# aliabdelkader/FusionTransformer

Measured on AMD Instinct MI355X. Metric: frames/sec fwd+bwd (SemanticKITTI synth), whole job, higher is better.
Workload: dtype f32

## Files before the change

fusiontransformer_amd/csrc/ftx_bn.hip:

```cpp
#include <cstdlib>
#include <map>
#include <mutex>
#include <utility>
#include "ftx_common.h"
#include "ftx_bn_eval_op.h"
#include "ftx_lastblock.h"

using namespace ftx;

namespace ftx {
namespace {
struct ScratchEntry {
  StreamScratch sc;
  void *owned;
};
std::mutex g_scratch_mu;
std::map<std::pair<int, hipStream_t>, ScratchEntry> g_scratch;

constexpr size_t scratch_counter_bytes() { return 512 * ((sizeof(uint32_t) * (1 + LB_MAX_GROUPS) + 511) / 512); }
constexpr size_t scratch_group_bytes() { return sizeof(double) * (size_t)LB_MAX_GROUPS * 2 * LB_MAX_COLS; }

int current_device() {
  int dev = 0;
  if (hipGetDevice(&dev) != hipSuccess) (void)hipGetLastError();
  return dev;
}
}

StreamScratch stream_scratch(hipStream_t st) {
  std::lock_guard<std::mutex> lock(g_scratch_mu);
  const auto key = std::make_pair(current_device(), st);
  auto it = g_scratch.find(key);
  if (it != g_scratch.end()) return it->second.sc;
  StreamScratch sc{nullptr, nullptr};
  hipStreamCaptureStatus cap = hipStreamCaptureStatusNone;
  if (hipStreamIsCapturing(st, &cap) == hipSuccess && cap != hipStreamCaptureStatusNone) {
    set_error("stream_scratch: first use of a stream inside a capture (attach a buffer, or run the op once on that stream, before capturing)");
    return sc;
  }
  (void)hipGetLastError();
  char *base = nullptr;
  if (hipMalloc((void **)&base, scratch_counter_bytes() + scratch_group_bytes()) != hipSuccess ||
      hipMemsetAsync(base, 0, scratch_counter_bytes(), st) != hipSuccess) {
    set_error("stream_scratch: cannot allocate the per-stream ticket buffer (%s)", hipGetErrorString(hipGetLastError()));
    if (base) (void)hipFree(base);
    return sc;
  }
  sc.counters = (uint32_t *)base;
  sc.gpart = (double *)(base + scratch_counter_bytes());
  g_scratch[key] = ScratchEntry{sc, base};
  return sc;
}
}

extern "C" size_t ftx_stream_scratch_bytes(void) { return scratch_counter_bytes() + scratch_group_bytes(); }

extern "C" int ftx_stream_scratch_attach(void *stream, void *buffer, size_t bytes) {
  FTX_REQUIRE(buffer && ((uintptr_t)buffer & 255) == 0, "ftx_stream_scratch_attach: the buffer must be non-null and 256-byte aligned");
  FTX_REQUIRE(bytes >= ftx_stream_scratch_bytes(), "ftx_stream_scratch_attach: %zu bytes < ftx_stream_scratch_bytes() = %zu", bytes, ftx_stream_scratch_bytes());
  hipStream_t st = (hipStream_t)stream;
  std::lock_guard<std::mutex> lock(g_scratch_mu);
  const auto key = std::make_pair(current_device(), st);
  if (hipMemsetAsync(buffer, 0, scratch_counter_bytes(), st) != hipSuccess) return check_launch("ftx_stream_scratch_attach memset");
  auto it = g_scratch.find(key);
  if (it != g_scratch.end() && it->second.owned) {
    if (hipStreamSynchronize(st) != hipSuccess) (void)hipGetLastError();
    (void)hipFree(it->second.owned);
  }
  StreamScratch sc{(uint32_t *)buffer, (double *)((char *)buffer + scratch_counter_bytes())};
  g_scratch[key] = ScratchEntry{sc, nullptr};
  return FTX_OK;
}

extern "C" int ftx_stream_scratch_reset(void *stream) {
  hipStream_t st = (hipStream_t)stream;
  std::lock_guard<std::mutex> lock(g_scratch_mu);
  auto it = g_scratch.find(std::make_pair(current_device(), st));
  if (it == g_scratch.end()) return FTX_OK;
  if (hipMemsetAsync(it->second.sc.counters, 0, scratch_counter_bytes(), st) != hipSuccess) return check_launch("ftx_stream_scratch_reset");
  return FTX_OK;
}

extern "C" int ftx_stream_scratch_release(void *stream) {
  hipStream_t st = (hipStream_t)stream;
  std::lock_guard<std::mutex> lock(g_scratch_mu);
  auto it = g_scratch.find(std::make_pair(current_device(), st));
  if (it == g_scratch.end()) return FTX_OK;
  if (hipStreamSynchronize(st) != hipSuccess) (void)hipGetLastError();
  if (it->second.owned) (void)hipFree(it->second.owned);
  g_scratch.erase(it);
  return FTX_OK;
}

static int bn_blocks(int64_t n) {
  constexpr int rows = 48, maxb = 2048;
  int64_t b = ceil_div(n, rows);
  if (b > maxb) b = maxb;
  if (b > LB_GROUP * LB_MAX_GROUPS) b = LB_GROUP * LB_MAX_GROUPS;
  if (b < 1) b = 1;
  return (int)b;
}

extern "C" size_t ftx_bn_workspace_bytes(int64_t n, int32_t c) {
  if (c <= 0) return 256;
  return sizeof(double) * (size_t)bn_blocks(n) * 2 * c + sizeof(double) * 2 * c;
}

__device__ inline float bn_affine(float x, float mean, float invstd, float gamma, float beta) {
  return __fmaf_rn(__fmul_rn(__fsub_rn(x, mean), invstd), gamma, beta);
}

struct FwdOp {
  __device__ static void eval(float x, float, float, float, float, float, float, int, double &q0, double &q1) {
    q0 = (double)x;
    q1 = (double)x * (double)x;
  }
};
struct BwdOp {
  __device__ static void eval(float x, float gy, float y, float mean, float invstd, float gamma, float beta, int relu, double &q0, double &q1) {
    if (relu == 2) y = bn_affine(x, mean, invstd, gamma, beta);
    float dy = (relu && !(y > 0.f)) ? 0.f : gy;
    q0 = (double)dy;
    q1 = (double)dy * (double)((x - mean) * invstd);
  }
};

template <class Op>
__global__ __launch_bounds__(256) void bn_partial_kernel(const float *__restrict__ x, const float *__restrict__ gy,
                                                         const float *__restrict__ y, const float *__restrict__ mean,
                                                         const float *__restrict__ invstd, const float *__restrict__ gamma,
                                                         const float *__restrict__ beta, int relu, int64_t n, int c,
                                                         double *part, StreamScratch sc) {
  extern __shared__ double sh[];
  const int c4 = c >> 2;
  const int RL = 256 / c4 > 0 ? 256 / c4 : 1;
  const int tid = threadIdx.x;
  const int cg = tid % c4, rl = tid / c4;
  const int64_t rows_per_block = ceil_div(n, (int64_t)gridDim.x);
  const int64_t r0 = (int64_t)blockIdx.x * rows_per_block;
  const int64_t r1 = (r0 + rows_per_block < n) ? r0 + rows_per_block : n;
  double s0[4] = {0, 0, 0, 0}, s1[4] = {0, 0, 0, 0};
  if (rl < RL) {
    float4 mu = make_float4(0, 0, 0, 0), is = mu, gm = mu, bt = mu;
    if (mean) {
      mu = *(const float4 *)&mean[cg * 4];
      is = *(const float4 *)&invstd[cg * 4];
    }
    if (relu == 2) {
      gm = *(const float4 *)&gamma[cg * 4];
      bt = *(const float4 *)&beta[cg * 4];
    }
    auto accumulate = [&](const float4 &xv, const float4 &gv, const float4 &yv) {
      double a, b;
      Op::eval(xv.x, gv.x, yv.x, mu.x, is.x, gm.x, bt.x, relu, a, b); s0[0] += a; s1[0] += b;
      Op::eval(xv.y, gv.y, yv.y, mu.y, is.y, gm.y, bt.y, relu, a, b); s0[1] += a; s1[1] += b;
      Op::eval(xv.z, gv.z, yv.z, mu.z, is.z, gm.z, bt.z, relu, a, b); s0[2] += a; s1[2] += b;
      Op::eval(xv.w, gv.w, yv.w, mu.w, is.w, gm.w, bt.w, relu, a, b); s0[3] += a; s1[3] += b;
    };
    const float4 zero4 = make_float4(0, 0, 0, 0);
    int64_t r = r0 + rl;
    for (; r + RL < r1; r += 2 * RL) {
      const int64_t o0 = r * c + cg * 4, o1 = (r + RL) * c + cg * 4;
      const float4 xa = *(const float4 *)&x[o0], xb = *(const float4 *)&x[o1];
      const float4 ga = gy ? *(const float4 *)&gy[o0] : zero4, gb = gy ? *(const float4 *)&gy[o1] : zero4;
      const float4 ya = y ? *(const float4 *)&y[o0] : zero4, yb = y ? *(const float4 *)&y[o1] : zero4;
      accumulate(xa, ga, ya);
      accumulate(xb, gb, yb);
    }
    for (; r < r1; r += RL) {
      const int64_t o0 = r * c + cg * 4;
      accumulate(*(const float4 *)&x[o0], gy ? *(const float4 *)&gy[o0] : zero4, y ? *(const float4 *)&y[o0] : zero4);
    }
#pragma unroll
    for (int v = 0; v < 4; ++v) {
      sh[(0 * RL + rl) * c + cg * 4 + v] = s0[v];
      sh[(1 * RL + rl) * c + cg * 4 + v] = s1[v];
    }
  }
  __syncthreads();
  for (int j = tid; j < 2 * c; j += 256) {
    int which = j / c, col = j - which * c;
    double s = 0;
    for (int q = 0; q < RL; ++q) s += sh[(which * RL + q) * c + col];
    lb_store(&part[((int64_t)blockIdx.x * 2 + which) * c + col], s);
  }
  __syncthreads();
  last_block_totals(part, (int)gridDim.x, c, sc, sh, StoreTotals{part + (int64_t)gridDim.x * 2 * c, c});
}

__device__ inline void bn_column_stats(double s, double ss, int64_t n, float eps, float &mean, float &invstd, double &var_out) {
  const double m = s / (double)n;
  double var = ss / (double)n - m * m;
  if (var < 0) var = 0;
  mean = (float)m;
  invstd = (float)(1.0 / sqrt(var + (double)eps));
  var_out = var;
}

__global__ __launch_bounds__(256) void bn_apply_fwd_kernel(const float *__restrict__ x, const float *__restrict__ res, const float *__restrict__ gamma,
                                                           const float *__restrict__ beta, const double *__restrict__ totals, float eps,
                                                           float momentum, float *__restrict__ running_mean, float *__restrict__ running_var,
                                                           float *__restrict__ save_mean, float *__restrict__ save_invstd, int64_t n, int c,
                                                           int relu, float *__restrict__ y) {
  const int c4 = c >> 2;
  const int RL = 256 / c4 > 0 ? 256 / c4 : 1;
  const int cg = threadIdx.x % c4, rl = threadIdx.x / c4;
  if (rl >= RL) return;
  const int col = cg * 4;
  float mu_[4], is_[4];
#pragma unroll
  for (int v = 0; v < 4; ++v) {
    double var;
    bn_column_stats(totals[col + v], totals[c + col + v], n, eps, mu_[v], is_[v], var);
    if (blockIdx.x == 0 && rl == 0) {
      save_mean[col + v] = mu_[v];
      save_invstd[col + v] = is_[v];
      if (running_mean) running_mean[col + v] = (1.f - momentum) * running_mean[col + v] + momentum * mu_[v];
      if (running_var) {
        const double unbiased = n > 1 ? var * (double)n / (double)(n - 1) : var;
        running_var[col + v] = (1.f - momentum) * running_var[col + v] + momentum * (float)unbiased;
      }
    }
  }
  const float4 mu = make_float4(mu_[0], mu_[1], mu_[2], mu_[3]), is = make_float4(is_[0], is_[1], is_[2], is_[3]);
  const float4 g = *(const float4 *)&gamma[col], b = *(const float4 *)&beta[col];
  auto one = [&](int64_t r) {
    const int64_t o = r * c + col;
    const float4 xv = *(const float4 *)&x[o];
    float4 ov;
    ov.x = bn_affine(xv.x, mu.x, is.x, g.x, b.x);
    ov.y = bn_affine(xv.y, mu.y, is.y, g.y, b.y);
    ov.z = bn_affine(xv.z, mu.z, is.z, g.z, b.z);
    ov.w = bn_affine(xv.w, mu.w, is.w, g.w, b.w);
    if (res) {
      const float4 rv = *(const float4 *)&res[o];
      ov.x += rv.x; ov.y += rv.y; ov.z += rv.z; ov.w += rv.w;
    }
    if (relu) {
      ov.x = ov.x > 0.f ? ov.x : 0.f; ov.y = ov.y > 0.f ? ov.y : 0.f;
      ov.z = ov.z > 0.f ? ov.z : 0.f; ov.w = ov.w > 0.f ? ov.w : 0.f;
    }
    *(float4 *)&y[o] = ov;
  };
  const int64_t stride = (int64_t)gridDim.x * RL;
  int64_t r = (int64_t)blockIdx.x * RL + rl;
  for (; r + stride < n; r += 2 * stride) {
    one(r);
    one(r + stride);
  }
  if (r < n) one(r);
}

static unsigned bn_apply_grid(int64_t n, int c) {
  const int c4 = c / 4;
  const int rl = 256 / c4 > 0 ? 256 / c4 : 1;
  int64_t g = ceil_div(n, 2 * (int64_t)rl);
  if (g > 4096) g = 4096;
  return (unsigned)(g < 1 ? 1 : g);
}

static int bn_check(const char *who, int64_t n, int c) {
  FTX_REQUIRE(n >= 0, "%s: n < 0", who);
  FTX_REQUIRE(c >= 4 && c % 4 == 0 && c <= 1024, "%s: c must be a multiple of 4 in [4,1024] (got %d)", who, c);
  return FTX_OK;
}

static size_t bn_partial_lds(int c) {
  int c4 = c / 4;
  int RL = 256 / c4 > 0 ? 256 / c4 : 1;
  return sizeof(double) * 2 * RL * c;
}

extern "C" int ftx_bn_train_fwd(const float *x, const float *residual, const float *gamma, const float *beta, float *running_mean,
                                float *running_var, float momentum, float eps, int64_t n, int32_t c, int32_t relu, float *y,
                                float *save_mean, float *save_invstd, void *workspace, size_t workspace_bytes, void *stream) {
  int rc = bn_check("ftx_bn_train_fwd", n, c);
  if (rc != FTX_OK) return rc;
  FTX_REQUIRE(n >= 1, "ftx_bn_train_fwd: needs at least one row");
  FTX_REQUIRE(x && gamma && beta && y && save_mean && save_invstd && workspace, "ftx_bn_train_fwd: null pointer");
  FTX_REQUIRE(c <= 512, "ftx_bn_train_fwd: c > 512 unsupported");
  if (workspace_bytes < ftx_bn_workspace_bytes(n, c)) {
    set_error("ftx_bn_train_fwd: workspace %zu < required %zu", workspace_bytes, ftx_bn_workspace_bytes(n, c));
    return FTX_EWORKSPACE;
  }
  hipStream_t st = (hipStream_t)stream;
  const StreamScratch sc = stream_scratch(st);
  if (!sc.counters) return FTX_ELAUNCH;
  const int nb = bn_blocks(n);
  double *part = (double *)workspace;
  bn_partial_kernel<FwdOp><<<nb, 256, bn_partial_lds(c), st>>>(x, nullptr, nullptr, nullptr, nullptr, nullptr, nullptr, 0, n, c, part, sc);
  bn_apply_fwd_kernel<<<bn_apply_grid(n, c), 256, 0, st>>>(x, residual, gamma, beta, part + (size_t)nb * 2 * c, eps, momentum, running_mean,
                                                           running_var, save_mean, save_invstd, n, c, relu, y);
  return check_launch("ftx_bn_train_fwd");
}

extern "C" int ftx_bn_train_fwd_totals(const float *x, const float *residual, const float *gamma, const float *beta, float *running_mean,
                                       float *running_var, float momentum, float eps, int64_t n, int32_t c, int32_t relu, float *y,
                                       float *save_mean, float *save_invstd, const double *totals, void *stream) {
  int rc = bn_check("ftx_bn_train_fwd_totals", n, c);
  if (rc != FTX_OK) return rc;
  FTX_REQUIRE(n >= 1, "ftx_bn_train_fwd_totals: needs at least one row");
  FTX_REQUIRE(x && gamma && beta && y && save_mean && save_invstd && totals, "ftx_bn_train_fwd_totals: null pointer");
  bn_apply_fwd_kernel<<<bn_apply_grid(n, c), 256, 0, (hipStream_t)stream>>>(x, residual, gamma, beta, totals, eps, momentum, running_mean,
                                                                            running_var, save_mean, save_invstd, n, c, relu, y);
  return check_launch("ftx_bn_train_fwd_totals");
}

__global__ void bn_apply_eval_kernel(const float *__restrict__ x, const float *__restrict__ res, const float *__restrict__ gamma,
                                     const float *__restrict__ beta, const float *__restrict__ rm, const float *__restrict__ rv, float eps,
                                     int64_t n, int c, int relu, float *__restrict__ y) {
  const int c4 = c >> 2;
  const int64_t total = n * c4;
  for (int64_t e = blockIdx.x * (int64_t)blockDim.x + threadIdx.x; e < total; e += (int64_t)gridDim.x * blockDim.x) {
    int col = (int)(e % c4) * 4;
    float4 xv = *(const float4 *)&x[e * 4];
    float o[4] = {xv.x, xv.y, xv.z, xv.w};
    float rr[4] = {0, 0, 0, 0};
    if (res) {
      float4 t = *(const float4 *)&res[e * 4];
      rr[0] = t.x; rr[1] = t.y; rr[2] = t.z; rr[3] = t.w;
    }
#pragma unroll
    for (int v = 0; v < 4; ++v) o[v] = bn_eval_elem(o[v], rm[col + v], rv[col + v], eps, gamma[col + v], beta[col + v], rr[v], relu);
    *(float4 *)&y[e * 4] = make_float4(o[0], o[1], o[2], o[3]);
  }
}

extern "C" int ftx_bn_eval_fwd(const float *x, const float *residual, const float *gamma, const float *beta, const float *running_mean,
                               const float *running_var, float eps, int64_t n, int32_t c, int32_t relu, float *y, void *stream) {
  int rc = bn_check("ftx_bn_eval_fwd", n, c);
  if (rc != FTX_OK) return rc;
  if (n == 0) return FTX_OK;
  FTX_REQUIRE(x && gamma && beta && running_mean && running_var && y, "ftx_bn_eval_fwd: null pointer");
  bn_apply_eval_kernel<<<grid_for(n * (c / 4), 256), 256, 0, (hipStream_t)stream>>>(x, residual, gamma, beta, running_mean, running_var, eps,
                                                                                     n, c, relu, y);
  return check_launch("ftx_bn_eval_fwd");
}

__global__ __launch_bounds__(256) void bn_apply_bwd_kernel(const float *__restrict__ gy, const float *__restrict__ x, const float *__restrict__ y,
                                                           const float *__restrict__ gamma, const float *__restrict__ beta,
                                                           const float *__restrict__ mean,
                                                           const float *__restrict__ invstd, const double *__restrict__ sums, int64_t n, int c,
                                                           int relu, float *__restrict__ gx, float *__restrict__ gres,
                                                           float *__restrict__ grad_gamma, float *__restrict__ grad_beta) {
  const int c4 = c >> 2;
  const int RL = 256 / c4 > 0 ? 256 / c4 : 1;
  const int cg = threadIdx.x % c4, rl = threadIdx.x / c4;
  if (rl >= RL) return;
  const int col = cg * 4;
  const float inv_n = 1.f / (float)n;
  float mu[4], is[4], gm[4], bt[4], sdy[4], sdyx[4];
#pragma unroll
  for (int v = 0; v < 4; ++v) {
    mu[v] = mean[col + v];
    is[v] = invstd[col + v];
    gm[v] = gamma[col + v];
    bt[v] = relu == 2 ? beta[col + v] : 0.f;
    sdy[v] = (float)sums[col + v] * inv_n;
    sdyx[v] = (float)sums[c + col + v] * inv_n;
    if (blockIdx.x == 0 && rl == 0) {
      if (grad_beta) grad_beta[col + v] = (float)sums[col + v];
      if (grad_gamma) grad_gamma[col + v] = (float)sums[c + col + v];
    }
  }
  auto one = [&](int64_t r) {
    const int64_t o = r * c + col;
    const float4 g4 = *(const float4 *)&gy[o];
    const float4 x4 = *(const float4 *)&x[o];
    float dy[4] = {g4.x, g4.y, g4.z, g4.w};
    const float xv[4] = {x4.x, x4.y, x4.z, x4.w};
    if (relu == 2) {
#pragma unroll
      for (int v = 0; v < 4; ++v)
        if (!(bn_affine(xv[v], mu[v], is[v], gm[v], bt[v]) > 0.f)) dy[v] = 0.f;
    } else if (relu) {
      const float4 y4 = *(const float4 *)&y[o];
      const float yv[4] = {y4.x, y4.y, y4.z, y4.w};
#pragma unroll
      for (int v = 0; v < 4; ++v)
        if (!(yv[v] > 0.f)) dy[v] = 0.f;
    }
    float ov[4];
#pragma unroll
    for (int v = 0; v < 4; ++v) {
      const float xhat = (xv[v] - mu[v]) * is[v];
      ov[v] = gm[v] * is[v] * (dy[v] - sdy[v] - xhat * sdyx[v]);
    }
    *(float4 *)&gx[o] = make_float4(ov[0], ov[1], ov[2], ov[3]);
    if (gres) *(float4 *)&gres[o] = make_float4(dy[0], dy[1], dy[2], dy[3]);
  };
  const int64_t stride = (int64_t)gridDim.x * RL;
  int64_t r = (int64_t)blockIdx.x * RL + rl;
  for (; r + stride < n; r += 2 * stride) {
    one(r);
    one(r + stride);
  }
  if (r < n) one(r);
}

extern "C" int ftx_bn_train_bwd(const float *grad_y, const float *x, const float *y, const float *gamma, const float *beta, const float *save_mean,
                                const float *save_invstd, int64_t n, int32_t c, int32_t relu, float *grad_x, float *grad_residual,
                                float *grad_gamma, float *grad_beta, void *workspace, size_t workspace_bytes, void *stream) {
  int rc = bn_check("ftx_bn_train_bwd", n, c);
  if (rc != FTX_OK) return rc;
  FTX_REQUIRE(n >= 1, "ftx_bn_train_bwd: needs at least one row");
  FTX_REQUIRE(grad_y && x && gamma && save_mean && save_invstd && grad_x && workspace, "ftx_bn_train_bwd: null pointer");
  const bool remask = relu && beta != nullptr && grad_residual == nullptr;
  FTX_REQUIRE(!relu || remask || y, "ftx_bn_train_bwd: relu needs the forward output y (or beta, when no residual went into it)");
  const int rmode = !relu ? 0 : (remask ? 2 : 1);
  FTX_REQUIRE(c <= 512, "ftx_bn_train_bwd: c > 512 unsupported");
  if (workspace_bytes < ftx_bn_workspace_bytes(n, c)) {
    set_error("ftx_bn_train_bwd: workspace %zu < required %zu", workspace_bytes, ftx_bn_workspace_bytes(n, c));
    return FTX_EWORKSPACE;
  }
  hipStream_t st = (hipStream_t)stream;
  const StreamScratch sc = stream_scratch(st);
  if (!sc.counters) return FTX_ELAUNCH;
  const int nb = bn_blocks(n);
  double *part = (double *)workspace;
  double *sums = part + (size_t)nb * 2 * c;
  bn_partial_kernel<BwdOp><<<nb, 256, bn_partial_lds(c), st>>>(x, grad_y, rmode == 1 ? y : nullptr, save_mean, save_invstd, gamma, beta, rmode, n, c, part, sc);
  bn_apply_bwd_kernel<<<bn_apply_grid(n, c), 256, 0, st>>>(grad_y, x, y, gamma, beta, save_mean, save_invstd, sums, n, c, rmode, grad_x, grad_residual,
                                                           grad_gamma, grad_beta);
  return check_launch("ftx_bn_train_bwd");
}

struct ColsumGeom {
  int c4w, rl, slab, chunks;
};
static ColsumGeom colsum_geom(int64_t rows, int cols) {
  ColsumGeom g;
  const int c4 = (cols + 3) / 4;
  g.c4w = c4 < 64 ? c4 : 64;
  g.rl = 256 / g.c4w;
  g.slab = g.c4w * 4;
  int64_t ch = ceil_div(rows, (int64_t)g.rl * 8);
  if (ch > 256) ch = 256;
  g.chunks = (int)(ch < 1 ? 1 : ch);
  return g;
}
extern "C" size_t ftx_colsum_workspace_bytes(int64_t rows, int32_t cols) {
  if (rows <= 0 || cols <= 0) return 256;
  return sizeof(double) * (size_t)colsum_geom(rows, cols).chunks * (size_t)cols + 256;
}

__global__ __launch_bounds__(256) void colsum_partial_kernel(const float *__restrict__ x, int64_t rows, int cols, int c4w, int RL,
                                                             double *__restrict__ part) {
  __shared__ double sh[1024];
  const int slab = c4w * 4;
  const int cq = threadIdx.x % c4w, rl = threadIdx.x / c4w;
  const int col = blockIdx.x * slab + cq * 4;
  const int64_t per = ceil_div(rows, (int64_t)gridDim.y);
  const int64_t r0 = (int64_t)blockIdx.y * per, r1 = r0 + per < rows ? r0 + per : rows;
  if (rl < RL) {
    double s[4] = {0, 0, 0, 0};
    if (col < cols) {
      int64_t r = r0 + rl;
      for (; r + RL < r1; r += 2 * RL) {
        const float4 a = *(const float4 *)&x[r * cols + col], b = *(const float4 *)&x[(r + RL) * cols + col];
        s[0] += (double)a.x; s[1] += (double)a.y; s[2] += (double)a.z; s[3] += (double)a.w;
        s[0] += (double)b.x; s[1] += (double)b.y; s[2] += (double)b.z; s[3] += (double)b.w;
      }
      for (; r < r1; r += RL) {
        const float4 a = *(const float4 *)&x[r * cols + col];
        s[0] += (double)a.x; s[1] += (double)a.y; s[2] += (double)a.z; s[3] += (double)a.w;
      }
    }
#pragma unroll
    for (int v = 0; v < 4; ++v) sh[rl * slab + cq * 4 + v] = s[v];
  }
  __syncthreads();
  for (int j = threadIdx.x; j < slab; j += 256) {
    const int c = blockIdx.x * slab + j;
    if (c < cols) {
      double t = 0;
      for (int q = 0; q < RL; ++q) t += sh[q * slab + j];
      part[(int64_t)blockIdx.y * cols + c] = t;
    }
  }
}
// ... 36 lines not shown
```

fusiontransformer_amd/csrc/ftx_lastblock.h:

```cpp
#pragma once
#include <assert.h>
#include "ftx_common.h"

#if defined(__HIP_DEVICE_COMPILE__) && !defined(__gfx950__) && !defined(__gfx942__) && !defined(__gfx90a__)
#error "ftx_lastblock.h relies on gfx9 (CDNA) memory-instruction semantics: sc1 write-through stores and vmcnt-counted store acknowledgements"
#endif

namespace ftx {

constexpr int LB_GROUP = 32;
constexpr int LB_MAX_GROUPS = 128;
constexpr int LB_MAX_COLS = 512;

struct StreamScratch {
  uint32_t *counters;
  double *gpart;
};
StreamScratch stream_scratch(hipStream_t st);

__device__ inline void lb_store(double *p, double v) { __hip_atomic_store(p, v, __ATOMIC_RELAXED, __HIP_MEMORY_SCOPE_AGENT); }
__device__ inline double lb_load(const double *p) { return __hip_atomic_load(p, __ATOMIC_RELAXED, __HIP_MEMORY_SCOPE_AGENT); }
__device__ inline uint32_t lb_ticket(uint32_t *p) { return __hip_atomic_fetch_add(p, 1u, __ATOMIC_RELAXED, __HIP_MEMORY_SCOPE_AGENT); }
__device__ inline void lb_stores_done() {
  asm volatile("s_waitcnt vmcnt(0)" ::: "memory");
  __syncthreads();
}

__device__ inline void lb_column_sums(const double *src, int nrows, int c2, double *slices, double *tot) {
  const int tid = threadIdx.x;
  auto strided_sum = [&](int j, int first, int step) {
    double s = 0;
    for (int base = first; base < nrows; base += 8 * step) {
      double v[8];
#pragma unroll
      for (int u = 0; u < 8; ++u) {
        const int r = base + u * step;
        v[u] = lb_load(&src[(int64_t)(r < nrows ? r : first) * c2 + j]);
        if (r >= nrows) v[u] = 0.0;
      }
#pragma unroll
      for (int u = 0; u < 8; ++u) s += v[u];
    }
    return s;
  };
  if (c2 <= 128) {
    const int R = 256 / c2, j = tid % c2, r = tid / c2;
    if (r < R) slices[r * c2 + j] = strided_sum(j, r, R);
    __syncthreads();
    if (tid < c2) {
      double t = 0;
      for (int q = 0; q < R; ++q) t += slices[q * c2 + tid];
      tot[tid] = t;
    }
  } else {
    for (int j = tid; j < c2; j += 256) tot[j] = strided_sum(j, 0, 1);
  }
  __syncthreads();
}

template <class Fin>
__device__ inline void last_block_totals(const double *part, int nb, int c, StreamScratch sc, double *lds, Fin fin) {
  __shared__ int s_last;
  const int tid = threadIdx.x, c2 = 2 * c;
  const int group = blockIdx.x / LB_GROUP, ngroups = (nb + LB_GROUP - 1) / LB_GROUP;
  const int g0 = group * LB_GROUP;
  const int gsize = nb - g0 < LB_GROUP ? nb - g0 : LB_GROUP;
  double *slices = lds, *tot = lds + 256;
  lb_stores_done();
  if (tid == 0) {
    const uint32_t ticket = lb_ticket(&sc.counters[1 + group]);
    assert(ticket < (uint32_t)gsize && "ftx: dirty BatchNorm ticket (a kernel died on this stream? call ftx_stream_scratch_reset)");
    s_last = ticket == (uint32_t)gsize - 1u;
  }
  __syncthreads();
  if (!s_last) return;
  lb_column_sums(part + (int64_t)g0 * c2, gsize, c2, slices, tot);
  for (int j = tid; j < c2; j += 256) lb_store(&sc.gpart[(int64_t)group * c2 + j], tot[j]);
  lb_stores_done();
  if (tid == 0) {
    __hip_atomic_store(&sc.counters[1 + group], 0u, __ATOMIC_RELAXED, __HIP_MEMORY_SCOPE_AGENT);
    const uint32_t ticket = lb_ticket(&sc.counters[0]);
    assert(ticket < (uint32_t)ngroups && "ftx: dirty BatchNorm group ticket (call ftx_stream_scratch_reset)");
    s_last = ticket == (uint32_t)ngroups - 1u;
  }
  __syncthreads();
  if (!s_last) return;
  if (tid == 0) __hip_atomic_store(&sc.counters[0], 0u, __ATOMIC_RELAXED, __HIP_MEMORY_SCOPE_AGENT);
  lb_column_sums(sc.gpart, ngroups, c2, slices, tot);
  for (int col = tid; col < c; col += 256) fin(col, tot[col], tot[c + col]);
}

struct StoreTotals {
  double *totals;
  int c;
  __device__ void operator()(int col, double s, double ss) const {
    totals[col] = s;
    totals[c + col] = ss;
  }
};

}
```

fusiontransformer_amd/csrc/ftx_spconv.hip:

```cpp
#include <cstring>
#include <cstdlib>
#include "ftx_common.h"
#include "ftx_bn_eval_op.h"
#include "ftx_mfma.h"
#include <rocprim/device/device_scan.hpp>
#include <rocprim/iterator/transform_iterator.hpp>

using namespace ftx;

struct IsValid {
  __host__ __device__ int32_t operator()(int32_t v) const { return v >= 0 ? 1 : 0; }
};

extern "C" size_t ftx_kernel_map_count_workspace_bytes(int64_t n_out, int32_t k) {
  if (n_out <= 0 || k <= 0) return 256;
  size_t bytes = 0;
  const int32_t *in = nullptr;
  int32_t *out = nullptr;
  auto it = rocprim::make_transform_iterator(in, IsValid());
  if (rocprim::exclusive_scan(nullptr, bytes, it, out, 0, (size_t)(n_out * k), rocprim::plus<int32_t>()) != hipSuccess) return 0;
  return bytes + 256;
}

__global__ void koff_kernel(const int32_t *__restrict__ nbr, const int32_t *__restrict__ scan, int64_t n_out, int k, int32_t *__restrict__ koff) {
// ... 442 lines not shown
  if (kvol == 27)
    spconv_reduce_bn_eval_kernel<27><<<(unsigned)g, 256, 0, st>>>(tmp, pos, n, co, residual, gamma, beta, running_mean, running_var, eps, relu, out);
  else
    spconv_reduce_bn_eval_kernel<8><<<(unsigned)g, 256, 0, st>>>(tmp, pos, n, co, residual, gamma, beta, running_mean, running_var, eps, relu, out);
  return check_launch("ftx_spconv_reduce_bn_eval");
}

template <int KVOL>
__global__ __launch_bounds__(256) void spconv_reduce_stats_kernel(const float *__restrict__ tmp, const int32_t *__restrict__ pos, int64_t n, int co,
                                                                  int kvol, float *__restrict__ out, double *part, StreamScratch sc) {
  extern __shared__ double sh[];
  const int cv = co >> 2;
  const int RL = 256 / cv;
  const int tid = threadIdx.x;
  const int cg = tid % cv, rl = tid / cv;
  const int64_t rows_per_block = ceil_div(n, (int64_t)gridDim.x);
  const int64_t r0 = (int64_t)blockIdx.x * rows_per_block;
  const int64_t r1 = (r0 + rows_per_block < n) ? r0 + rows_per_block : n;
  double s0[4] = {0, 0, 0, 0}, s1[4] = {0, 0, 0, 0};
  if (rl < RL) {
    const int j = cg * 4;
    for (int64_t r = r0 + rl; r < r1; r += RL) {
      float4 acc = make_float4(0.f, 0.f, 0.f, 0.f);
      if (KVOL > 0) {
        int32_t p[KVOL > 0 ? KVOL : 1];
#pragma unroll
        for (int k = 0; k < KVOL; ++k) p[k] = pos[(int64_t)k * n + r];
#pragma unroll
        for (int k = 0; k < KVOL; ++k) {
          if (p[k] >= 0) {
            float4 v = *(const float4 *)&tmp[(int64_t)p[k] * co + j];
            acc.x += v.x; acc.y += v.y; acc.z += v.z; acc.w += v.w;
          }
        }
      } else {
        for (int k = 0; k < kvol; ++k) {
          int32_t q = pos[(int64_t)k * n + r];
          if (q >= 0) {
            float4 v = *(const float4 *)&tmp[(int64_t)q * co + j];
            acc.x += v.x; acc.y += v.y; acc.z += v.z; acc.w += v.w;
          }
        }
      }
      *(float4 *)&out[r * co + j] = acc;
      s0[0] += (double)acc.x; s1[0] += (double)acc.x * (double)acc.x;
      s0[1] += (double)acc.y; s1[1] += (double)acc.y * (double)acc.y;
      s0[2] += (double)acc.z; s1[2] += (double)acc.z * (double)acc.z;
      s0[3] += (double)acc.w; s1[3] += (double)acc.w * (double)acc.w;
    }
#pragma unroll
    for (int v = 0; v < 4; ++v) {
      sh[(0 * RL + rl) * co + j + v] = s0[v];
      sh[(1 * RL + rl) * co + j + v] = s1[v];
    }
  }
  __syncthreads();
  for (int e = tid; e < 2 * co; e += 256) {
    int which = e / co, col = e - which * co;
    double s = 0;
    for (int q = 0; q < RL; ++q) s += sh[(which * RL + q) * co + col];
    lb_store(&part[((int64_t)blockIdx.x * 2 + which) * co + col], s);
  }
  __syncthreads();
  last_block_totals(part, (int)gridDim.x, co, sc, sh, StoreTotals{part + (int64_t)gridDim.x * 2 * co, co});
}

extern "C" int32_t ftx_spconv_reduce_stats_blocks(int64_t n, int32_t co) {
  if (n <= 0 || co < 4) return 1;
  const int rl = 256 / (co / 4) > 0 ? 256 / (co / 4) : 1;
  int64_t b = ceil_div(n, 2 * rl);
  if (b > 2048) b = 2048;
  return (int32_t)(b < 1 ? 1 : b);
}

extern "C" int ftx_spconv_reduce_stats(const float *tmp, const int32_t *pos, int64_t n, int32_t co, int32_t kvol, float *out, double *part,
                                       int32_t nb, void *stream) {
  FTX_REQUIRE(n >= 1 && kvol >= 1 && co >= 4 && co % 4 == 0 && co <= 512, "ftx_spconv_reduce_stats: bad size (co must be a multiple of 4 in [4, 512])");
  FTX_REQUIRE(pos && out && part, "ftx_spconv_reduce_stats: null pointer");
  FTX_REQUIRE(nb == ftx_spconv_reduce_stats_blocks(n, co), "ftx_spconv_reduce_stats: nb must come from ftx_spconv_reduce_stats_blocks");
  hipStream_t st = (hipStream_t)stream;
  const StreamScratch sc = stream_scratch(st);
  if (!sc.counters) return FTX_ELAUNCH;
  const int rl = 256 / (co / 4);
  const size_t lds = sizeof(double) * 2 * rl * co;
  if (kvol == 27)
    spconv_reduce_stats_kernel<27><<<nb, 256, lds, st>>>(tmp, pos, n, co, kvol, out, part, sc);
  else if (kvol == 8)
    spconv_reduce_stats_kernel<8><<<nb, 256, lds, st>>>(tmp, pos, n, co, kvol, out, part, sc);
  else
    spconv_reduce_stats_kernel<0><<<nb, 256, lds, st>>>(tmp, pos, n, co, kvol, out, part, sc);
  return check_launch("ftx_spconv_reduce_stats");
}

constexpr int WG_BR = 32;
constexpr int WG_ROUND = 1024;

template <int N> struct FragLoad;
template <> struct FragLoad<1> { static __device__ __forceinline__ void ld(const float *p, float (&f)[1]) { f[0] = *p; } };
template <> struct FragLoad<2> { static __device__ __forceinline__ void ld(const float *p, float (&f)[2]) { float2 v = *(const float2 *)p; f[0] = v.x; f[1] = v.y; } };
template <> struct FragLoad<3> { static __device__ __forceinline__ void ld(const float *p, float (&f)[3]) { f[0] = p[0]; f[1] = p[1]; f[2] = p[2]; } };
template <> struct FragLoad<4> { static __device__ __forceinline__ void ld(const float *p, float (&f)[4]) { float4 v = *(const float4 *)p; f[0] = v.x; f[1] = v.y; f[2] = v.z; f[3] = v.w; } };

template <int MI, int NI, int WMG, int WNG>
__global__ __launch_bounds__(256) void pairs_wgrad_kernel(const float *__restrict__ A, int64_t rows_a, const int32_t *__restrict__ idx_a,
                                                          const float *__restrict__ G, int64_t rows_g, const int32_t *__restrict__ idx_g,
                                                          const int32_t *__restrict__ koff, int ca, int cg, int kvol, int tile_len,
                                                          float *__restrict__ part, float *__restrict__ dW, int n_dense) {
  constexpr int TM = 32 * MI * WMG, TN = 32 * NI * WNG, KS = 4 / (WMG * WNG);
  constexpr int STAGE = WG_BR * (TM + TN);
  constexpr int RED = KS > 1 ? MI * NI * 1024 * WMG * WNG : 0;
  constexpr int LDSF = STAGE > RED ? STAGE : RED;
  __shared__ __attribute__((aligned(16))) float lds[LDSF];
  __shared__ int32_t s_ia[WG_ROUND], s_ig[WG_ROUND];
  __shared__ uint8_t s_ok[WG_ROUND];
  __shared__ int s_tile[4];
  __shared__ int s_bad;
  float *As = lds, *Gs = lds + WG_BR * TM;

  const int tid = threadIdx.x, wave = tid >> 6, lane = tid & 63;
  const int half = lane >> 5, l31 = lane & 31;
  const int wq = wave % (WMG * WNG), ks = wave / (WMG * WNG);
  const int wm = wq % WMG, wn = wq / WMG;
  if (tid < 64) {
    const int b = blockIdx.x;
    int c = 0;
    if (tid < kvol) c = koff ? koff[tid + 1] - koff[tid] : n_dense;
    int nt = (c + tile_len - 1) / tile_len;
    int incl = nt;
#pragma unroll
    for (int off = 1; off < 64; off <<= 1) {
      int v = __shfl_up(incl, off, 64);
      if (tid >= off) incl += v;
    }
    int excl = incl - nt;
    bool mine = (tid < kvol) && b >= excl && b < incl;
    unsigned long long msk = __ballot(mine);
    if (mine) {
      int t = b - excl;
      int first = (koff ? koff[tid] : 0) + t * tile_len;
      int left = c - t * tile_len;
      s_tile[0] = tid;
      s_tile[1] = first;
      s_tile[2] = first + (left > tile_len ? tile_len : left);
      s_tile[3] = nt;
    }
    if (msk == 0ull && tid == 0) s_tile[0] = -1;
  }
  __syncthreads();
  const int k = s_tile[0];
  if (k < 0) return;
  const int m0 = blockIdx.y * TM, n0 = blockIdx.z * TN;
  const int lo = s_tile[1], hi = s_tile[2];
  const bool single = s_tile[3] == 1;

  f32x16 acc[MI][NI];
#pragma unroll
  for (int i = 0; i < MI; ++i)
#pragma unroll
    for (int j = 0; j < NI; ++j)
#pragma unroll
      for (int g = 0; g < 16; ++g) acc[i][j][g] = 0.f;

  constexpr int QA = TM / 32, QG = TN / 32;
  float4 ra0[QA], rg0[QG], ra1[QA], rg1[QG];
  int rbase = lo, rend = lo;
  int pra[QA], prg[QG], ca_off[QA], cg_off[QG];
#pragma unroll
// ... 259 lines not shown
```

fusiontransformer_amd/csrc/ftx_stn.hip:

```cpp
#include "ftx_common.h"
#include "ftx_lastblock.h"

#pragma clang fp contract(off)

using namespace ftx;

namespace {

constexpr int AFF_MAX_B = 128;
constexpr int AFF_MAX_BLOCKS = 1024;

struct AffSrc {
  const float *p;
  int64_t sb, sc, sy, sx;
  int b, c, ih, iw;
};

struct AffTap {
  int x0, y0;
  float ex, fx, ey, fy;
  float xn, yn;
  bool live;
  bool nan;
};
// ... 19 lines not shown
    t.ey = (yf + 1.f) - iy;
    t.fy = iy - yf;
  }
  return t;
}

__device__ inline void aff_corners(const AffSrc &S, int f, int ch, const AffTap &t, float &v00, float &v01, float &v10, float &v11) {
  const float *pl = S.p + (int64_t)f * S.sb + (int64_t)ch * S.sc;
  const bool xa = t.x0 >= 0, xb = t.x0 + 1 < S.iw, ya = t.y0 >= 0, yb = t.y0 + 1 < S.ih;
  const int64_t o = (int64_t)t.y0 * S.sy + (int64_t)t.x0 * S.sx;
  v00 = (xa && ya) ? pl[o] : 0.f;
  v01 = (xb && ya) ? pl[o + S.sx] : 0.f;
  v10 = (xa && yb) ? pl[o + S.sy] : 0.f;
  v11 = (xb && yb) ? pl[o + S.sy + S.sx] : 0.f;
}

__device__ inline float aff_value(const AffSrc &S, int f, int ch, const AffTap &t) {
  if (!t.live) return t.nan ? __builtin_nanf("") : 0.f;
  float v00, v01, v10, v11;
  aff_corners(S, f, ch, t, v00, v01, v10, v11);
  return ((v00 * (t.ex * t.ey) + v01 * (t.fx * t.ey)) + v10 * (t.ex * t.fy)) + v11 * (t.fx * t.fy);
}

__device__ inline bool aff_point(const int64_t *__restrict__ img_idx, const int32_t *__restrict__ pb, int64_t i, int b, int H, int W, int &f,
                                 int &r, int &col) {
  const int64_t rr = img_idx[i * 2], cc = img_idx[i * 2 + 1];
  f = pb[i];
  r = (int)rr;
  col = (int)cc;
  return f >= 0 && f < b && rr >= 0 && rr < H && cc >= 0 && cc < W;
}

__global__ __launch_bounds__(256) void aff_sample_fwd_kernel(AffSrc S, const float *__restrict__ theta, int oh, int ow, float *__restrict__ out) {
  const int64_t P = (int64_t)oh * ow, total = (int64_t)S.b * P;
  for (int64_t p = blockIdx.x * (int64_t)blockDim.x + threadIdx.x; p < total; p += (int64_t)gridDim.x * blockDim.x) {
    const int f = (int)(p / P);
    const int64_t q = p - (int64_t)f * P;
    const int r = (int)(q / ow), col = (int)(q - (int64_t)r * ow);
    const AffTap t = aff_tap(theta + f * 6, r, col, oh, ow, S.ih, S.iw);
    for (int ch = 0; ch < S.c; ++ch) out[((int64_t)f * S.c + ch) * P + q] = aff_value(S, f, ch, t);
  }
}

__global__ __launch_bounds__(256) void aff_lift_fwd_kernel(AffSrc S, const float *__restrict__ theta, const int64_t *__restrict__ img_idx,
                                                           const int32_t *__restrict__ pb, int64_t n, int H, int W, float *__restrict__ out) {
  const int64_t total = n * S.c;
  for (int64_t e = blockIdx.x * (int64_t)blockDim.x + threadIdx.x; e < total; e += (int64_t)gridDim.x * blockDim.x) {
    const int64_t i = e / S.c;
    const int ch = (int)(e - i * S.c);
    int f, r, col;
    float v = 0.f;
    if (aff_point(img_idx, pb, i, S.b, H, W, f, r, col)) v = aff_value(S, f, ch, aff_tap(theta + f * 6, r, col, H, W, S.ih, S.iw));
    out[e] = v;
  }
}

__global__ __launch_bounds__(256) void aff_lift_cells_kernel(const float *__restrict__ theta, const int64_t *__restrict__ img_idx,
                                                             const int32_t *__restrict__ pb, int64_t n, int b, int ih, int iw, int H, int W,
                                                             int32_t *__restrict__ cells) {
  for (int64_t i = blockIdx.x * (int64_t)blockDim.x + threadIdx.x; i < n; i += (int64_t)gridDim.x * blockDim.x) {
    int f, r, col;
    int32_t key = -1;
    if (aff_point(img_idx, pb, i, b, H, W, f, r, col)) {
      const AffTap t = aff_tap(theta + f * 6, r, col, H, W, ih, iw);
      if (t.live) key = (int32_t)(((int64_t)f * (ih + 1) + (t.y0 + 1)) * (iw + 1) + (t.x0 + 1));
    }
    cells[i] = key;
  }
}

struct StoreTheta {
  float *grad_theta;
  int c3;
  __device__ void operator()(int col, double lo, double hi) const {
    grad_theta[col] = (float)lo;
    grad_theta[c3 + col] = (float)hi;
  }
};

template <bool POINTS>
__global__ __launch_bounds__(256) void aff_theta_kernel(AffSrc S, const float *__restrict__ theta, const float *__restrict__ go,
                                                        const int64_t *__restrict__ img_idx, const int32_t *__restrict__ pb, int64_t n, int H, int W,
                                                        int G, int bpf, double *__restrict__ part, StreamScratch sc, float *__restrict__ grad_theta) {
  __shared__ double lds[256 + 6 * AFF_MAX_B];
  const int tid = threadIdx.x;
  const int f = blockIdx.x / bpf, k = blockIdx.x - f * bpf;
  const int per = 256 / G, sub = tid & (G - 1);
  const int64_t P = (int64_t)H * W;
  double acc[6] = {0, 0, 0, 0, 0, 0};
  for (int64_t base = (int64_t)k * per; base < n; base += (int64_t)bpf * per) {
    const int64_t item = base + tid / G;
    bool ok = item < n;
    int r = 0, col = 0;
    if (POINTS) {
      int pf = -1;
      ok = ok && aff_point(img_idx, pb, item, S.b, H, W, pf, r, col) && pf == f;
    } else if (ok) {
      r = (int)(item / W);
      col = (int)(item - (int64_t)r * W);
    }
    AffTap t;
    t.live = false;
    if (ok) t = aff_tap(theta + f * 6, r, col, H, W, S.ih, S.iw);
    float gix = 0.f, giy = 0.f;
    if (ok && t.live) {
      for (int ch = sub; ch < S.c; ch += G) {
        float v00, v01, v10, v11;
        aff_corners(S, f, ch, t, v00, v01, v10, v11);
        const float g = POINTS ? go[item * S.c + ch] : go[((int64_t)f * S.c + ch) * P + item];
        gix += ((v01 - v00) * t.ey + (v11 - v10) * t.fy) * g;
        giy += ((v10 - v00) * t.ex + (v11 - v01) * t.fx) * g;
      }
    }
    for (int off = 1; off < G; off <<= 1) {
      gix += __shfl_xor(gix, off, 64);
      giy += __shfl_xor(giy, off, 64);
    }
    if (sub == 0 && ok && t.live) {
      const double gx = (double)(gix * ((float)S.iw / 2.f)), gy = (double)(giy * ((float)S.ih / 2.f));
      acc[0] += gx * t.xn; acc[1] += gx * t.yn; acc[2] += gx;
      acc[3] += gy * t.xn; acc[4] += gy * t.yn; acc[5] += gy;
    }
  }
  const int lane = tid & 63, wave = tid >> 6;
#pragma unroll
  for (int q = 0; q < 6; ++q) {
    double v = acc[q];
#pragma unroll
    for (int off = 32; off > 0; off >>= 1) v += __shfl_down(v, off, 64);
    if (lane == 0) lds[wave * 6 + q] = v;
  }
  __syncthreads();
  const int c2 = 6 * S.b;
  double *row = part + (int64_t)blockIdx.x * c2;
  for (int j = tid; j < c2; j += 256) {
    const int jf = j / 6, q = j - jf * 6;
    lb_store(&row[j], jf == f ? ((lds[q] + lds[6 + q]) + lds[12 + q]) + lds[18 + q] : 0.0);
  }
  __syncthreads();
  last_block_totals(part, (int)gridDim.x, 3 * S.b, sc, lds, StoreTheta{grad_theta, 3 * S.b});
}

__global__ __launch_bounds__(256) void aff_lift_bwd_src_kernel(AffSrc S, float *__restrict__ gs, const float *__restrict__ theta,
                                                               const int64_t *__restrict__ img_idx, const float *__restrict__ go,
                                                               const int32_t *__restrict__ order, const int32_t *__restrict__ seg_off, int H,
                                                               int W, int chan_inner) {
  const int64_t total = (int64_t)S.b * S.c * S.ih * S.iw;
  for (int64_t e = blockIdx.x * (int64_t)blockDim.x + threadIdx.x; e < total; e += (int64_t)gridDim.x * blockDim.x) {
    int f, ch, y, x;
    int64_t q = e;
    if (chan_inner) {
      ch = (int)(q % S.c); q /= S.c;
      x = (int)(q % S.iw); q /= S.iw;
      y = (int)(q % S.ih);
      f = (int)(q / S.ih);
    } else {
      x = (int)(q % S.iw); q /= S.iw;
      y = (int)(q % S.ih); q /= S.ih;
      ch = (int)(q % S.c);
      f = (int)(q / S.c);
    }
    float acc = 0.f;
#pragma unroll
    for (int s = 0; s < 4; ++s) {
      const int ky = y + 1 - (s >> 1), kx = x + 1 - (s & 1);
      const int64_t key = ((int64_t)f * (S.ih + 1) + ky) * (S.iw + 1) + kx;
      const int lo = seg_off[key], hi = seg_off[key + 1];
// ... 145 lines not shown
```

Before: 151.4.

## Unroll BN loops by four and parallelize last-block column reduction across slices

BN stat-partial, apply and backward kernels now issue four independent float4 row loads before computing, raising memory-level parallelism, and the grid sizes are reduced to match. The last-block reduction splits the column sums across multiple row slices even for wide channel counts, instead of one thread per column walking all rows serially. A single-group fast path skips the second-level global handover. LDS sizing is adjusted for the larger slice buffer, which raises shared-memory use per block and costs some occupancy.

```diff
diff --git a/fusiontransformer_amd/csrc/ftx_bn.hip b/fusiontransformer_amd/csrc/ftx_bn.hip
--- a/fusiontransformer_amd/csrc/ftx_bn.hip
+++ b/fusiontransformer_amd/csrc/ftx_bn.hip
@@ -93,7 +93,7 @@
 }
 
 static int bn_blocks(int64_t n) {
-  constexpr int rows = 48, maxb = 2048;
+  constexpr int rows = 32, maxb = 1024;
   int64_t b = ceil_div(n, rows);
   if (b > maxb) b = maxb;
   if (b > LB_GROUP * LB_MAX_GROUPS) b = LB_GROUP * LB_MAX_GROUPS;
@@ -159,17 +159,30 @@
     };
     const float4 zero4 = make_float4(0, 0, 0, 0);
     int64_t r = r0 + rl;
-    for (; r + RL < r1; r += 2 * RL) {
-      const int64_t o0 = r * c + cg * 4, o1 = (r + RL) * c + cg * 4;
-      const float4 xa = *(const float4 *)&x[o0], xb = *(const float4 *)&x[o1];
-      const float4 ga = gy ? *(const float4 *)&gy[o0] : zero4, gb = gy ? *(const float4 *)&gy[o1] : zero4;
-      const float4 ya = y ? *(const float4 *)&y[o0] : zero4, yb = y ? *(const float4 *)&y[o1] : zero4;
-      accumulate(xa, ga, ya);
-      accumulate(xb, gb, yb);
-    }
-    for (; r < r1; r += RL) {
-      const int64_t o0 = r * c + cg * 4;
-      accumulate(*(const float4 *)&x[o0], gy ? *(const float4 *)&gy[o0] : zero4, y ? *(const float4 *)&y[o0] : zero4);
+    for (; r + 3 * RL < r1; r += 4 * RL) {
+      float4 xv[4], gv[4], yv[4];
+#pragma unroll
+      for (int u = 0; u < 4; ++u) {
+        const int64_t o = (r + u * RL) * c + cg * 4;
+        xv[u] = *(const float4 *)&x[o];
+        gv[u] = gy ? *(const float4 *)&gy[o] : zero4;
+        yv[u] = y ? *(const float4 *)&y[o] : zero4;
+      }
+#pragma unroll
+      for (int u = 0; u < 4; ++u) accumulate(xv[u], gv[u], yv[u]);
+    }
+    if (r < r1) {
+      float4 xv[3], gv[3], yv[3];
+#pragma unroll
+      for (int u = 0; u < 3; ++u) {
+        const int64_t o = (r + u * RL < r1 ? r + u * RL : r) * c + cg * 4;
+        xv[u] = *(const float4 *)&x[o];
+        gv[u] = gy ? *(const float4 *)&gy[o] : zero4;
+        yv[u] = y ? *(const float4 *)&y[o] : zero4;
+      }
+#pragma unroll
+      for (int u = 0; u < 3; ++u)
+        if (r + u * RL < r1) accumulate(xv[u], gv[u], yv[u]);
     }
 #pragma unroll
     for (int v = 0; v < 4; ++v) {
@@ -224,16 +237,13 @@
   }
   const float4 mu = make_float4(mu_[0], mu_[1], mu_[2], mu_[3]), is = make_float4(is_[0], is_[1], is_[2], is_[3]);
   const float4 g = *(const float4 *)&gamma[col], b = *(const float4 *)&beta[col];
-  auto one = [&](int64_t r) {
-    const int64_t o = r * c + col;
-    const float4 xv = *(const float4 *)&x[o];
+  auto one = [&](int64_t o, const float4 &xv, const float4 &rv) {
     float4 ov;
     ov.x = bn_affine(xv.x, mu.x, is.x, g.x, b.x);
     ov.y = bn_affine(xv.y, mu.y, is.y, g.y, b.y);
     ov.z = bn_affine(xv.z, mu.z, is.z, g.z, b.z);
     ov.w = bn_affine(xv.w, mu.w, is.w, g.w, b.w);
     if (res) {
-      const float4 rv = *(const float4 *)&res[o];
       ov.x += rv.x; ov.y += rv.y; ov.z += rv.z; ov.w += rv.w;
     }
     if (relu) {
@@ -243,19 +253,25 @@
     *(float4 *)&y[o] = ov;
   };
   const int64_t stride = (int64_t)gridDim.x * RL;
-  int64_t r = (int64_t)blockIdx.x * RL + rl;
-  for (; r + stride < n; r += 2 * stride) {
-    one(r);
-    one(r + stride);
-  }
-  if (r < n) one(r);
+  for (int64_t r = (int64_t)blockIdx.x * RL + rl; r < n; r += 4 * stride) {
+    float4 xv[4], rv[4];
+#pragma unroll
+    for (int u = 0; u < 4; ++u) {
+      const int64_t o = (r + u * stride < n ? r + u * stride : r) * c + col;
+      xv[u] = *(const float4 *)&x[o];
+      rv[u] = res ? *(const float4 *)&res[o] : make_float4(0.f, 0.f, 0.f, 0.f);
+    }
+#pragma unroll
+    for (int u = 0; u < 4; ++u)
+      if (r + u * stride < n) one((r + u * stride) * c + col, xv[u], rv[u]);
+  }
 }
 
 static unsigned bn_apply_grid(int64_t n, int c) {
   const int c4 = c / 4;
   const int rl = 256 / c4 > 0 ? 256 / c4 : 1;
-  int64_t g = ceil_div(n, 2 * (int64_t)rl);
-  if (g > 4096) g = 4096;
+  int64_t g = ceil_div(n, 4 * (int64_t)rl);
+  if (g > 2048) g = 2048;
   return (unsigned)(g < 1 ? 1 : g);
 }
 
@@ -268,7 +284,8 @@
 static size_t bn_partial_lds(int c) {
   int c4 = c / 4;
   int RL = 256 / c4 > 0 ? 256 / c4 : 1;
-  return sizeof(double) * 2 * RL * c;
+  const int rows = 2 * RL * c, handover = lb_lds_doubles(c);
+  return sizeof(double) * (rows > handover ? rows : handover);
 }
 
 extern "C" int ftx_bn_train_fwd(const float *x, const float *residual, const float *gamma, const float *beta, float *running_mean,
@@ -363,10 +380,7 @@
       if (grad_gamma) grad_gamma[col + v] = (float)sums[c + col + v];
     }
   }
-  auto one = [&](int64_t r) {
-    const int64_t o = r * c + col;
-    const float4 g4 = *(const float4 *)&gy[o];
-    const float4 x4 = *(const float4 *)&x[o];
+  auto one = [&](int64_t o, const float4 &g4, const float4 &x4, const float4 &y4) {
     float dy[4] = {g4.x, g4.y, g4.z, g4.w};
     const float xv[4] = {x4.x, x4.y, x4.z, x4.w};
     if (relu == 2) {
@@ -374,7 +388,6 @@
       for (int v = 0; v < 4; ++v)
         if (!(bn_affine(xv[v], mu[v], is[v], gm[v], bt[v]) > 0.f)) dy[v] = 0.f;
     } else if (relu) {
-      const float4 y4 = *(const float4 *)&y[o];
       const float yv[4] = {y4.x, y4.y, y4.z, y4.w};
 #pragma unroll
       for (int v = 0; v < 4; ++v)
@@ -390,12 +403,19 @@
     if (gres) *(float4 *)&gres[o] = make_float4(dy[0], dy[1], dy[2], dy[3]);
   };
   const int64_t stride = (int64_t)gridDim.x * RL;
-  int64_t r = (int64_t)blockIdx.x * RL + rl;
-  for (; r + stride < n; r += 2 * stride) {
-    one(r);
-    one(r + stride);
-  }
-  if (r < n) one(r);
+  for (int64_t r = (int64_t)blockIdx.x * RL + rl; r < n; r += 4 * stride) {
+    float4 g4[4], x4[4], y4[4];
+#pragma unroll
+    for (int u = 0; u < 4; ++u) {
+      const int64_t o = (r + u * stride < n ? r + u * stride : r) * c + col;
+      g4[u] = *(const float4 *)&gy[o];
+      x4[u] = *(const float4 *)&x[o];
+      y4[u] = relu == 1 ? *(const float4 *)&y[o] : make_float4(0.f, 0.f, 0.f, 0.f);
+    }
+#pragma unroll
+    for (int u = 0; u < 4; ++u)
+      if (r + u * stride < n) one((r + u * stride) * c + col, g4[u], x4[u], y4[u]);
+  }
 }
 
 extern "C" int ftx_bn_train_bwd(const float *grad_y, const float *x, const float *y, const float *gamma, const float *beta, const float *save_mean,
diff --git a/fusiontransformer_amd/csrc/ftx_lastblock.h b/fusiontransformer_amd/csrc/ftx_lastblock.h
--- a/fusiontransformer_amd/csrc/ftx_lastblock.h
+++ b/fusiontransformer_amd/csrc/ftx_lastblock.h
@@ -26,46 +26,72 @@
   __syncthreads();
 }
 
-__device__ inline void lb_column_sums(const double *src, int nrows, int c2, double *slices, double *tot) {
-  const int tid = threadIdx.x;
-  auto strided_sum = [&](int j, int first, int step) {
-    double s = 0;
-    for (int base = first; base < nrows; base += 8 * step) {
-      double v[8];
+constexpr int LB_INFLIGHT = 8;
+__host__ __device__ constexpr int lb_slices(int c2) {
+  if (c2 <= 128) return 256 / c2;
+  int s = 1;
+  while (2 * s * c2 <= 1024) s *= 2;
+  return s;
+}
+__host__ __device__ constexpr int lb_lds_doubles(int c) { return (2 * c <= 128 ? 256 : 1024) + 2 * c; }
+
+template <int IT, int RW>
+__device__ __forceinline__ void lb_slice_sums(const double *src, int nrows, int c2, int S, double *slices) {
+  const int nitems = S * c2, rps = (nrows + S - 1) / S;
+  for (int w0 = threadIdx.x; w0 < nitems; w0 += 256 * IT) {
+    int sl[IT], col[IT];
+    double acc[IT];
 #pragma unroll
-      for (int u = 0; u < 8; ++u) {
-        const int r = base + u * step;
-        v[u] = lb_load(&src[(int64_t)(r < nrows ? r : first) * c2 + j]);
-        if (r >= nrows) v[u] = 0.0;
-      }
+    for (int i = 0; i < IT; ++i) {
+      const int w = w0 + 256 * i < nitems ? w0 + 256 * i : w0;
+      sl[i] = w / c2;
+      col[i] = w - sl[i] * c2;
+      acc[i] = 0;
+    }
+    for (int k0 = 0; k0 < rps; k0 += RW) {
+      double v[IT][RW];
 #pragma unroll
-      for (int u = 0; u < 8; ++u) s += v[u];
+      for (int i = 0; i < IT; ++i)
+#pragma unroll
+        for (int u = 0; u < RW; ++u) {
+          const int r = sl[i] + (k0 + u) * S;
+          v[i][u] = lb_load(src + (uint32_t)((r < nrows ? r : 0) * c2 + col[i]));
+          if (r >= nrows) v[i][u] = 0.0;
+        }
+#pragma unroll
+      for (int i = 0; i < IT; ++i)
+#pragma unroll
+        for (int u = 0; u < RW; ++u) acc[i] += v[i][u];
     }
-    return s;
-  };
-  if (c2 <= 128) {
-    const int R = 256 / c2, j = tid % c2, r = tid / c2;
-    if (r < R) slices[r * c2 + j] = strided_sum(j, r, R);
-    __syncthreads();
-    if (tid < c2) {
-      double t = 0;
-      for (int q = 0; q < R; ++q) t += slices[q * c2 + tid];
-      tot[tid] = t;
-    }
-  } else {
-    for (int j = tid; j < c2; j += 256) tot[j] = strided_sum(j, 0, 1);
+#pragma unroll
+    for (int i = 0; i < IT; ++i)
+      if (w0 + 256 * i < nitems) slices[w0 + 256 * i] = acc[i];
+  }
+}
+
+__device__ __forceinline__ void lb_column_sums(const double *src, int nrows, int c2, double *slices, double *tot) {
+  const int tid = threadIdx.x, S = lb_slices(c2);
+  if ((nrows + S - 1) / S <= LB_INFLIGHT / 2 && S * c2 > 256)
+    lb_slice_sums<2, LB_INFLIGHT / 2>(src, nrows, c2, S, slices);
+  else
+    lb_slice_sums<1, LB_INFLIGHT>(src, nrows, c2, S, slices);
+  __syncthreads();
+  for (int j = tid; j < c2; j += 256) {
+    double t = 0;
+    for (int q = 0; q < S; ++q) t += slices[q * c2 + j];
+    tot[j] = t;
   }
   __syncthreads();
 }
 
 template <class Fin>
-__device__ inline void last_block_totals(const double *part, int nb, int c, StreamScratch sc, double *lds, Fin fin) {
+__device__ __forceinline__ void last_block_totals(const double *part, int nb, int c, StreamScratch sc, double *lds, Fin fin) {
   __shared__ int s_last;
   const int tid = threadIdx.x, c2 = 2 * c;
   const int group = blockIdx.x / LB_GROUP, ngroups = (nb + LB_GROUP - 1) / LB_GROUP;
   const int g0 = group * LB_GROUP;
   const int gsize = nb - g0 < LB_GROUP ? nb - g0 : LB_GROUP;
-  double *slices = lds, *tot = lds + 256;
+  double *slices = lds, *tot = lds + (c2 <= 128 ? 256 : 1024);
   lb_stores_done();
   if (tid == 0) {
     const uint32_t ticket = lb_ticket(&sc.counters[1 + group]);
@@ -75,6 +101,11 @@
   __syncthreads();
   if (!s_last) return;
   lb_column_sums(part + (int64_t)g0 * c2, gsize, c2, slices, tot);
+  if (ngroups == 1) {
+    if (tid == 0) __hip_atomic_store(&sc.counters[1], 0u, __ATOMIC_RELAXED, __HIP_MEMORY_SCOPE_AGENT);
+    for (int col = tid; col < c; col += 256) fin(col, tot[col], tot[c + col]);
+    return;
+  }
   for (int j = tid; j < c2; j += 256) lb_store(&sc.gpart[(int64_t)group * c2 + j], tot[j]);
   lb_stores_done();
   if (tid == 0) {
diff --git a/fusiontransformer_amd/csrc/ftx_spconv.hip b/fusiontransformer_amd/csrc/ftx_spconv.hip
--- a/fusiontransformer_amd/csrc/ftx_spconv.hip
+++ b/fusiontransformer_amd/csrc/ftx_spconv.hip
@@ -548,7 +548,7 @@
   const StreamScratch sc = stream_scratch(st);
   if (!sc.counters) return FTX_ELAUNCH;
   const int rl = 256 / (co / 4);
-  const size_t lds = sizeof(double) * 2 * rl * co;
+  const size_t lds = sizeof(double) * (2 * rl * co > lb_lds_doubles(co) ? 2 * rl * co : lb_lds_doubles(co));
   if (kvol == 27)
     spconv_reduce_stats_kernel<27><<<nb, 256, lds, st>>>(tmp, pos, n, co, kvol, out, part, sc);
   else if (kvol == 8)
diff --git a/fusiontransformer_amd/csrc/ftx_stn.hip b/fusiontransformer_amd/csrc/ftx_stn.hip
--- a/fusiontransformer_amd/csrc/ftx_stn.hip
+++ b/fusiontransformer_amd/csrc/ftx_stn.hip
@@ -125,7 +125,7 @@
 __global__ __launch_bounds__(256) void aff_theta_kernel(AffSrc S, const float *__restrict__ theta, const float *__restrict__ go,
                                                         const int64_t *__restrict__ img_idx, const int32_t *__restrict__ pb, int64_t n, int H, int W,
                                                         int G, int bpf, double *__restrict__ part, StreamScratch sc, float *__restrict__ grad_theta) {
-  __shared__ double lds[256 + 6 * AFF_MAX_B];
+  __shared__ double lds[lb_lds_doubles(3 * AFF_MAX_B)];
   const int tid = threadIdx.x;
   const int f = blockIdx.x / bpf, k = blockIdx.x - f * bpf;
   const int per = 256 / G, sub = tid & (G - 1);
```

After: 147.1. 2.8% lower.
